# jkflying/opencalibration

Hardware: AMD Instinct MI355X
Metric: images/sec end-to-end (extract+match+relax) on synthetic aerial grid; LM iters/sec (higher is better)
Workload: dtype f32 (extract) + fp4 0/1 bits, f32 accumulate, exact (match) + f64 (RANSAC, relax)

## Files before the change

opencalibration_amd/csrc/match.hip:

```cpp
#include "ctx.hpp"

#include <algorithm>
#include <unordered_map>
#include <vector>

namespace
{

constexpr int BLOCK = 256;
constexpr uint32_t KEY_SHIFT = 20;
constexpr uint32_t KEY_MASK = (1u << KEY_SHIFT) - 1;

__device__ __forceinline__ uint32_t med3_u32(uint32_t a, uint32_t b, uint32_t c)
{
    uint32_t r;
    asm("v_med3_u32 %0, %1, %2, %3" : "=v"(r) : "v"(a), "v"(b), "v"(c));
    return r;
}

__device__ __forceinline__ uint32_t bcnt_acc(uint32_t x, uint32_t acc)
{
    uint32_t r;
    asm("v_bcnt_u32_b32 %0, %1, %2" : "=v"(r) : "v"(x), "v"(acc));
    return r;
}

template <int QPT>
__global__ __launch_bounds__(BLOCK) void hamming_2nn_kernel(const uint32_t *__restrict__ desc,
                                                            const uint64_t *__restrict__ img_off,
                                                            const uint32_t *__restrict__ img_n,
                                                            const ochip_pair *__restrict__ pairs,
                                                            const uint64_t *__restrict__ out_off,
                                                            ochip_match *__restrict__ out, uint32_t chunks_per_pair)
{
    const uint32_t pair = blockIdx.x / chunks_per_pair;
    const uint32_t chunk = blockIdx.x - pair * chunks_per_pair;
    const ochip_pair pr = pairs[pair];
    const uint32_t n1 = img_n[pr.image_1], n2 = img_n[pr.image_2];
    const uint32_t q0 = chunk * (BLOCK * QPT);
    if (q0 >= n1)
        return;
    const uint32_t *__restrict__ Q = desc + img_off[pr.image_1] * 16;
    const uint32_t *__restrict__ R = desc + img_off[pr.image_2] * 16;

    uint32_t q[QPT][16];
    uint32_t best[QPT], second[QPT];
#pragma unroll
    for (int j = 0; j < QPT; j++)
    {
        uint32_t qi = q0 + j * BLOCK + threadIdx.x;
        qi = qi < n1 ? qi : n1 - 1;
        const uint4 *src = reinterpret_cast<const uint4 *>(Q + (size_t)qi * 16);
#pragma unroll
        for (int v = 0; v < 4; v++)
        {
            const uint4 t = src[v];
            q[j][4 * v + 0] = t.x;
            q[j][4 * v + 1] = t.y;
            q[j][4 * v + 2] = t.z;
            q[j][4 * v + 3] = t.w;
        }
        best[j] = 0xFFFFFFFFu;
        second[j] = 0xFFFFFFFFu;
    }

    auto load_row = [&](uint32_t (&rw)[16], uint32_t k) {
        const uint32_t kk = k < n2 ? k : n2 - 1;
        const uint32_t *__restrict__ r = R + (size_t)kk * 16;
#pragma unroll
        for (int w = 0; w < 16; w++)
            rw[w] = r[w];
    };
    auto score_row = [&](const uint32_t (&rw)[16], uint32_t k) {
#pragma unroll
        for (int j = 0; j < QPT; j++)
        {
            uint32_t cnt = 0;
#pragma unroll
            for (int w = 0; w < 16; w++)
                cnt = bcnt_acc(q[j][w] ^ rw[w], cnt);
            const uint32_t key = (cnt << KEY_SHIFT) | k;
            second[j] = med3_u32(best[j], second[j], key);
            best[j] = best[j] < key ? best[j] : key;
        }
    };
    if (n2 > 0)
    {
        uint32_t ra[16], rb[16];
        load_row(ra, 0);
        uint32_t k = 0;
        for (; k + 1 < n2; k += 2)
        {
            load_row(rb, k + 1);
            score_row(ra, k);
            load_row(ra, k + 2);
            score_row(rb, k + 1);
        }
        if (k < n2)
            score_row(ra, k);
    }

    ochip_match *__restrict__ o = out + out_off[pair];
#pragma unroll
    for (int j = 0; j < QPT; j++)
    {
        const uint32_t qi = q0 + j * BLOCK + threadIdx.x;
        if (qi < n1)
        {
            ochip_match m;
            m.best_k = best[j] & KEY_MASK;
            m.best_count = (uint16_t)(best[j] >> KEY_SHIFT);
            m.second_count = second[j] == 0xFFFFFFFFu ? (uint16_t)OCHIP_NO_SECOND : (uint16_t)(second[j] >> KEY_SHIFT);
            o[qi] = m;
        }
    }
}

struct sym_job
{
    uint32_t a, b;
    uint64_t off_ab, off_ba;
    uint64_t part_off;
};

__device__ __forceinline__ void top2_merge(uint32_t &b, uint32_t &s, uint32_t ob, uint32_t os)
{
    const uint32_t lo = b < ob ? b : ob, hi = b < ob ? ob : b, ms = s < os ? s : os;
    b = lo;
    s = hi < ms ? hi : ms;
}

__global__ __launch_bounds__(BLOCK) void hamming_2nn_sym_kernel(const uint32_t *__restrict__ desc, const uint64_t *__restrict__ img_off,
                                                                const uint32_t *__restrict__ img_n, const sym_job *__restrict__ jobs,
                                                                ochip_match *__restrict__ out, uint2 *__restrict__ part,
                                                                uint32_t chunks_per_pair)
{
    __shared__ uint32_t T[4][16 * 65];
    const uint32_t pair = blockIdx.x / chunks_per_pair;
    const uint32_t chunk = blockIdx.x - pair * chunks_per_pair;
    const sym_job jb = jobs[pair];
    const uint32_t nA = img_n[jb.a], nB = img_n[jb.b];
    const uint32_t q0 = chunk * BLOCK;
    if (q0 >= nA)
        return;
    const int lane = threadIdx.x & 63, wv = threadIdx.x >> 6;
    if (q0 + wv * 64 >= nA)
        return;
    const uint32_t *__restrict__ Q = desc + img_off[jb.a] * 16;
    const uint32_t *__restrict__ R = desc + img_off[jb.b] * 16;
    const uint32_t qi = q0 + threadIdx.x;
    const bool q_valid = qi < nA;
    uint32_t q[16];
    {
        const uint4 *src = reinterpret_cast<const uint4 *>(Q + (size_t)(q_valid ? qi : nA - 1) * 16);
#pragma unroll
        for (int v = 0; v < 4; v++)
        {
            const uint4 t = src[v];
            q[4 * v + 0] = t.x;
            q[4 * v + 1] = t.y;
            q[4 * v + 2] = t.z;
            q[4 * v + 3] = t.w;
        }
    }
    uint32_t best = 0xFFFFFFFFu, second = 0xFFFFFFFFu;
    auto load_row = [&](uint32_t (&rw)[16], uint32_t k) {
        const uint32_t kk = k < nB ? k : nB - 1;
        const uint32_t *__restrict__ r = R + (size_t)kk * 16;
#pragma unroll
        for (int w = 0; w < 16; w++)
            rw[w] = r[w];
    };
    auto count_row = [&](const uint32_t (&rw)[16]) {
        uint32_t cnt = 0;
#pragma unroll
        for (int w = 0; w < 16; w++)
            cnt = bcnt_acc(q[w] ^ rw[w], cnt);
        return cnt;
    };
    uint32_t *Tw = T[wv];
    const uint32_t n_tiles = (nB + 31) / 32;
    for (uint32_t jt = 0; jt < n_tiles; jt++)
    {
        const uint32_t k0 = jt * 32;
        uint32_t ra[16], rb[16];
        load_row(ra, k0);
#pragma unroll 4
        for (uint32_t j = 0; j < 32; j += 2)
        {
            load_row(rb, k0 + j + 1);
            const uint32_t c0 = count_row(ra);
            load_row(ra, k0 + j + 2);
            const uint32_t c1 = count_row(rb);
            const uint32_t ka = k0 + j, kb = ka + 1;
            if (ka < nB)
            {
                const uint32_t key = (c0 << KEY_SHIFT) | ka;
                second = med3_u32(best, second, key);
                best = best < key ? best : key;
            }
            if (kb < nB)
            {
                const uint32_t key = (c1 << KEY_SHIFT) | kb;
                second = med3_u32(best, second, key);
                best = best < key ? best : key;
            }
            const uint32_t s0 = (q_valid && ka < nB) ? c0 : 0xFFFFu, s1 = (q_valid && kb < nB) ? c1 : 0xFFFFu;
            Tw[(j >> 1) * 65 + lane] = s0 | (s1 << 16);
        }
        __builtin_amdgcn_fence(__ATOMIC_SEQ_CST, "wavefront");
        __builtin_amdgcn_wave_barrier();
        uint32_t cb = 0xFFFFFFFFu, cs = 0xFFFFFFFFu;
        {
            const uint32_t jj = lane & 31, half = lane >> 5;
            const uint32_t *col = Tw + (jj >> 1) * 65 + half * 32;
            const uint32_t sh = (jj & 1) * 16;
            const uint32_t qbase = q0 + wv * 64 + half * 32;
#pragma unroll 8
            for (uint32_t i = 0; i < 32; i++)
            {
                const uint32_t c = (col[i] >> sh) & 0xFFFFu;
                const uint32_t key = (c << KEY_SHIFT) | (qbase + i);
                cs = med3_u32(cb, cs, key);
                cb = cb < key ? cb : key;
            }
            const uint32_t ob = (uint32_t)__shfl_xor((int)cb, 32), os = (uint32_t)__shfl_xor((int)cs, 32);
            top2_merge(cb, cs, ob, os);
            const uint32_t ref = k0 + jj;
            if (half == 0 && ref < nB)
                part[jb.part_off + (size_t)(chunk * 4 + wv) * nB + ref] = make_uint2(cb, cs);
        }
        __builtin_amdgcn_fence(__ATOMIC_SEQ_CST, "wavefront");
        __builtin_amdgcn_wave_barrier();
    }
    if (q_valid)
    {
        ochip_match m;
        m.best_k = best & KEY_MASK;
        m.best_count = (uint16_t)(best >> KEY_SHIFT);
        m.second_count = second == 0xFFFFFFFFu ? (uint16_t)OCHIP_NO_SECOND : (uint16_t)(second >> KEY_SHIFT);
        out[jb.off_ab + qi] = m;
    }
}

__global__ __launch_bounds__(BLOCK) void sym_merge_kernel(const sym_job *__restrict__ jobs, const uint32_t *__restrict__ img_n,
                                                          const uint2 *__restrict__ part, ochip_match *__restrict__ out)
{
    const sym_job jb = jobs[blockIdx.x];
    const uint32_t nA = img_n[jb.a], nB = img_n[jb.b];
    const uint32_t r = blockIdx.y * BLOCK + threadIdx.x;
    if (r >= nB)
        return;
    uint32_t b = 0xFFFFFFFFu, s = 0xFFFFFFFFu;
    const uint32_t tiles = (nA + 63) / 64;
    for (uint32_t c = 0; c < tiles; c++)
    {
        const uint2 p = part[jb.part_off + (size_t)c * nB + r];
        top2_merge(b, s, p.x, p.y);
    }
    ochip_match m;
    m.best_k = b & KEY_MASK;
    m.best_count = (uint16_t)(b >> KEY_SHIFT);
    m.second_count = (s >> KEY_SHIFT) == 0xFFFu ? (uint16_t)OCHIP_NO_SECOND : (uint16_t)(s >> KEY_SHIFT);
    out[jb.off_ba + r] = m;
}

typedef int v8i __attribute__((ext_vector_type(8)));
typedef float v16f __attribute__((ext_vector_type(16)));
constexpr uint32_t MFMA_MAX_REFS = 8192;
constexpr int MFMA_QT = 2;
constexpr int MFMA_QUERIES = 4 * 32 * MFMA_QT;

__global__ __launch_bounds__(256) void expand_fp4_kernel(const uint32_t *__restrict__ desc, uint64_t first, uint64_t n,
                                                         uint32_t *__restrict__ fp4, float *__restrict__ negpop,
                                                         uint32_t *__restrict__ pop)
{
    const uint64_t f = first + (uint64_t)blockIdx.x * 4 + (threadIdx.x >> 6);
    if (f >= first + n)
        return;
    const int j = threadIdx.x & 63;
    const uint32_t x = (desc[f * 16 + (j >> 2)] >> (8 * (j & 3))) & 0xFFu;
    uint32_t t = (x | (x << 12)) & 0x000F000Fu;
    t = (t | (t << 6)) & 0x03030303u;
    t = (t | (t << 3)) & 0x11111111u;
    fp4[f * 64 + j] = t << 1;
    uint32_t c = (uint32_t)__popc(x);
    for (int off = 32; off >= 1; off >>= 1)
        c += (uint32_t)__shfl_xor((int)c, off);
    if (j == 0)
    {
        pop[f] = c;
        negpop[f] = (float)((512 - (int)c) * 8192);
    }
}

__device__ __forceinline__ float med3_f32(float a, float b, float c)
{
    return __builtin_amdgcn_fmed3f(a, b, c);
}
__device__ __forceinline__ float max_f32(float a, float b)
{
    return __int_as_float(max(__float_as_int(a), __float_as_int(b)));
}

__global__ __launch_bounds__(256) void hamming_2nn_mfma_kernel(const uint4 *__restrict__ fp4, const float *__restrict__ negpop,
                                                               const uint32_t *__restrict__ pop,
                                                               const uint64_t *__restrict__ img_off,
                                                               const uint32_t *__restrict__ img_n,
                                                               const ochip_pair *__restrict__ pairs,
                                                               const uint64_t *__restrict__ out_off,
                                                               ochip_match *__restrict__ out, uint32_t chunks_per_pair)
{
    constexpr int TR = 64;
    __shared__ uint4 tileA[2][TR * 17];
    __shared__ float tileC[2][TR];
    const uint32_t pair = blockIdx.x / chunks_per_pair;
    const uint32_t chunk = blockIdx.x - pair * chunks_per_pair;
    const ochip_pair pr = pairs[pair];
    const uint32_t n1 = img_n[pr.image_1], n2 = img_n[pr.image_2];
    const uint32_t q0 = chunk * MFMA_QUERIES;
    if (q0 >= n1 || n2 == 0)
        return;
    const uint64_t off1 = img_off[pr.image_1], off2 = img_off[pr.image_2];
    const int tid = threadIdx.x, lane = tid & 63, wv = tid >> 6, r = lane & 31, h = lane >> 5;
    constexpr int QT = MFMA_QT;
    v8i Bq[QT][8];
#pragma unroll
    for (int t = 0; t < QT; t++)
    {
        uint32_t qi = q0 + wv * (32 * QT) + t * 32 + r;
        qi = qi < n1 ? qi : n1 - 1;
        const uint4 *src = fp4 + (off1 + qi) * 16;
#pragma unroll
        for (int sidx = 0; sidx < 8; sidx++)
        {
            const uint4 v = src[2 * sidx + h];
            Bq[t][sidx] = v8i{(int)v.x, (int)v.y, (int)v.z, (int)v.w, 0, 0, 0, 0};
        }
    }
    float best[QT], second[QT];
#pragma unroll
    for (int t = 0; t < QT; t++)
        best[t] = second[t] = -1.0f;
    const uint32_t n_tiles = (n2 + TR - 1) / TR;
    const uint4 *gsrc = fp4 + off2 * 16 + tid;
    const float *gneg = negpop + off2 + (tid & 63);
    const int st0 = (tid >> 4) * 17 + (tid & 15);
    auto load_tile = [&](uint32_t jt, uint4 (&p)[4], float &c) {
        if ((jt + 1) * TR <= n2)
        {
#pragma unroll
            for (int i = 0; i < 4; i++)
                p[i] = gsrc[(size_t)jt * (TR * 16) + 256 * i];
            c = gneg[jt * TR] + (float)(8191 - (int)(jt * TR + (uint32_t)(tid & 63)));
        }
        else
        {
#pragma unroll
            for (int i = 0; i < 4; i++)
            {
                const uint32_t k = jt * TR + ((uint32_t)tid >> 4) + 16 * i;
                p[i] = fp4[(off2 + (k < n2 ? k : n2 - 1)) * 16 + (tid & 15)];
            }
            const uint32_t kc = jt * TR + (uint32_t)(tid & 63);
            c = kc < n2 ? negpop[off2 + kc] + (float)(8191 - (int)kc) : -1e9f;
        }
    };
    auto put_tile = [&](int buf, const uint4 (&p)[4], float c) {
#pragma unroll
        for (int i = 0; i < 4; i++)
            tileA[buf][st0 + 16 * 17 * i] = p[i];
        if (tid < TR)
            tileC[buf][tid] = c;
    };
    {
        uint4 p[4];
        float c;
        load_tile(0, p, c);
        put_tile(0, p, c);
    }
    __syncthreads();
    uint4 nx[2][4];
    float nc[2] = {0.0f, 0.0f};
#pragma unroll
    for (int q = 0; q < 2; q++)
#pragma unroll
        for (int i = 0; i < 4; i++)
            nx[q][i] = make_uint4(0, 0, 0, 0);
    if (n_tiles > 1)
        load_tile(1, nx[1], nc[1]);
    auto tile = [&](uint32_t jt, uint4 (&mine)[4], float &mine_c, uint4 (&ahead)[4], float &ahead_c) {
        const int cur = (int)(jt & 1);
        const bool more = jt + 1 < n_tiles;
        if (jt + 2 < n_tiles)
            load_tile(jt + 2, ahead, ahead_c);
        v16f acc[2][QT];
#pragma unroll
        for (int sub = 0; sub < 2; sub++)
        {
#pragma unroll
            for (int gidx = 0; gidx < 4; gidx++)
            {
                const float4 c4 = *reinterpret_cast<const float4 *>(&tileC[cur][32 * sub + 8 * gidx + 4 * h]);
                acc[sub][0][4 * gidx + 0] = c4.x;
                acc[sub][0][4 * gidx + 1] = c4.y;
                acc[sub][0][4 * gidx + 2] = c4.z;
                acc[sub][0][4 * gidx + 3] = c4.w;
            }
#pragma unroll
            for (int t = 1; t < QT; t++)
                acc[sub][t] = acc[sub][0];
        }
        typedef int v4i __attribute__((ext_vector_type(4)));
#pragma unroll
        for (int half = 0; half < 2; half++)
        {
            v4i a[2][4];
#pragma unroll
            for (int sub = 0; sub < 2; sub++)
            {
                const uint4 *arow = &tileA[cur][(32 * sub + r) * 17 + h + 8 * half];
#pragma unroll
                for (int sidx = 0; sidx < 4; sidx++)
                {
                    const uint4 t = arow[2 * sidx];
                    a[sub][sidx] = v4i{(int)t.x, (int)t.y, (int)t.z, (int)t.w};
                }
            }
            asm volatile("" : "+v"(a[0][0]), "+v"(a[0][1]), "+v"(a[0][2]), "+v"(a[0][3]), "+v"(a[1][0]), "+v"(a[1][1]), "+v"(a[1][2]), "+v"(a[1][3]));
#pragma unroll
            for (int sidx = 0; sidx < 4; sidx++)
#pragma unroll
                for (int sub = 0; sub < 2; sub++)
                {
                    const v8i A = v8i{a[sub][sidx].x, a[sub][sidx].y, a[sub][sidx].z, a[sub][sidx].w, 0, 0, 0, 0};
#pragma unroll
                    for (int t = 0; t < QT; t++)
                        acc[sub][t] = __builtin_amdgcn_mfma_scale_f32_32x32x64_f8f6f4(A, Bq[t][4 * half + sidx], acc[sub][t], 4, 4, 0, 141, 0, 127);
                }
        }
#pragma unroll
        for (int sub = 0; sub < 2; sub++)
#pragma unroll
            for (int i = 0; i < 16; i++)
            {
#pragma unroll
                for (int t = 0; t < QT; t++)
                {
                    second[t] = med3_f32(best[t], second[t], acc[sub][t][i]);
                    best[t] = max_f32(best[t], acc[sub][t][i]);
                }
            }
        if (more)
            put_tile(cur ^ 1, mine, mine_c);
        __syncthreads();
    };
    for (uint32_t jt = 0; jt < n_tiles; jt += 2)
    {
        tile(jt, nx[1], nc[1], nx[0], nc[0]);
        if (jt + 1 < n_tiles)
            tile(jt + 1, nx[0], nc[0], nx[1], nc[1]);
    }
    ochip_match *__restrict__ o = out + out_off[pair];
#pragma unroll
    for (int t = 0; t < QT; t++)
    {
        const float ob = __shfl_xor(best[t], 32), os = __shfl_xor(second[t], 32);
        const float hi = fmaxf(best[t], ob), lo = fminf(best[t], ob), ms = fmaxf(second[t], os);
        const float b2 = fmaxf(lo, ms);
        const uint32_t qi = q0 + wv * (32 * QT) + t * 32 + r;
        if (h == 0 && qi < n1)
        {
            const uint32_t pq = pop[off1 + qi];
            const int kb = (int)hi;
            ochip_match m;
            m.best_k = 8191u - ((uint32_t)kb & 8191u);
            m.best_count = (uint16_t)(pq + 512u - ((uint32_t)kb >> 13));
            m.second_count = b2 < 0.0f ? (uint16_t)OCHIP_NO_SECOND : (uint16_t)(pq + 512u - ((uint32_t)(int)b2 >> 13));
            o[qi] = m;
        }
    }
}

}

extern "C"
{

int ochip_match_launch(ochip_ctx *ctx, const ochip_pair *pairs, uint32_t n_pairs, const uint64_t *out_offset,
                       uint64_t out_total)
{
    if (!ctx)
        return OCHIP_EINVAL;
    if (n_pairs && (!pairs || !out_offset))
        return ochip_fail(ctx, OCHIP_EINVAL, "pairs/out_offset is NULL");
    if (!ctx->desc_dev)
        return ochip_fail(ctx, OCHIP_ESTATE, "ochip_descriptors_reserve has not been called");
    OCHIP_HIP(ctx, hipSetDevice(ctx->device));
    ctx->match_out_total = out_total;
    if (n_pairs == 0)
        return OCHIP_OK;

    uint32_t max_n1 = 0;
    for (uint32_t p = 0; p < n_pairs; p++)
    {
        const ochip_pair &pr = pairs[p];
        if (pr.image_1 >= ctx->n_images || pr.image_2 >= ctx->n_images || !ctx->img_set[pr.image_1] ||
            !ctx->img_set[pr.image_2])
            return ochip_fail(ctx, OCHIP_ESTATE, "pair %u references an image that was not uploaded", p);
        if (ctx->img_n[pr.image_2] > KEY_MASK)
            return ochip_fail(ctx, OCHIP_EINVAL, "image %u has %u descriptors; the kernel supports <= %u", pr.image_2,
                              ctx->img_n[pr.image_2], KEY_MASK);
        if (out_offset[p] + ctx->img_n[pr.image_1] > out_total)
            return ochip_fail(ctx, OCHIP_EINVAL, "out_offset[%u] + n1 exceeds out_total", p);
        max_n1 = ctx->img_n[pr.image_1] > max_n1 ? ctx->img_n[pr.image_1] : max_n1;
    }

    static const bool use_mfma = !ochip_test_hook("popcount_match");
    std::vector<ochip_pair> mfma_pairs;
    std::vector<uint64_t> mfma_off;
    uint32_t mfma_max_n1 = 0;
    std::vector<char> claimed(n_pairs, 0);
    if (use_mfma)
        for (uint32_t p = 0; p < n_pairs; p++)
        {
            const uint32_t na = ctx->img_n[pairs[p].image_1], nb = ctx->img_n[pairs[p].image_2];
            if (na == 0 || nb == 0 || nb > MFMA_MAX_REFS)
                continue;
            claimed[p] = 1;
            mfma_pairs.push_back(pairs[p]);
            mfma_off.push_back(out_offset[p]);
            mfma_max_n1 = std::max(mfma_max_n1, na);
            ctx->match_computed += (uint64_t)na * nb;
            ctx->match_delivered += (uint64_t)na * nb;
        }
    const uint32_t n_mfma = (uint32_t)mfma_pairs.size();
    constexpr bool use_sym = true;
    std::vector<sym_job> sym;
    std::vector<ochip_pair> single_pairs;
    std::vector<uint64_t> single_off;
    uint64_t part_total = 0, part_max = 0;
    uint32_t sym_max_na = 0, sym_max_nb = 0;
    std::vector<uint32_t> sym_groups{0};
    {
        std::unordered_map<uint64_t, uint32_t> first;
        if (use_sym)
            for (uint32_t p = 0; p < n_pairs; p++)
                if (!claimed[p])
                    first.emplace(((uint64_t)pairs[p].image_1 << 32) | pairs[p].image_2, p);
        for (uint32_t p = 0; p < n_pairs; p++)
        {
            if (claimed[p])
                continue;
            const uint32_t a = pairs[p].image_1, b = pairs[p].image_2;
            const uint32_t na = ctx->img_n[a], nb = ctx->img_n[b];
            static const uint64_t cap_bytes = getenv("OCHIP_MATCH_SYM_CAP_MB") ? (uint64_t)atoll(getenv("OCHIP_MATCH_SYM_CAP_MB")) << 20 : (8ull << 30);
            const uint64_t need = (uint64_t)((na + 63) / 64) * nb;
            if (use_sym && a != b && na > 0 && nb > 0 && need * sizeof(uint2) <= cap_bytes)
            {
                auto it = first.find(((uint64_t)b << 32) | a);
                if (it != first.end() && it->second != p && !claimed[it->second])
                {
                    claimed[p] = claimed[it->second] = 1;
                    if ((part_total + need) * sizeof(uint2) > cap_bytes)
                    {
                        sym_groups.push_back((uint32_t)sym.size());
                        part_total = 0;
                    }
                    sym.push_back(sym_job{a, b, out_offset[p], out_offset[it->second], part_total});
                    part_total += need;
                    part_max = std::max(part_max, part_total);
                    ctx->match_computed += (uint64_t)na * nb;
                    ctx->match_delivered += 2 * (uint64_t)na * nb;
                    sym_max_na = std::max(sym_max_na, na);
                    sym_max_nb = std::max(sym_max_nb, nb);
                    continue;
                }
            }
            claimed[p] = 1;
            ctx->match_computed += (uint64_t)na * nb;
            ctx->match_delivered += (uint64_t)na * nb;
            single_pairs.push_back(pairs[p]);
            single_off.push_back(out_offset[p]);
        }
    }
    const uint32_t n_single = (uint32_t)single_pairs.size(), n_sym = (uint32_t)sym.size();
    uint32_t max_n1_single = 0;
    for (const ochip_pair &pr : single_pairs)
        max_n1_single = std::max(max_n1_single, ctx->img_n[pr.image_1]);

    OCHIP_TRY(ochip_upload_image_tables(ctx));
    OCHIP_TRY(ctx->pairs_dev.ensure(ctx, n_single + n_mfma));
    OCHIP_TRY(ctx->out_off_dev.ensure(ctx, n_single + n_mfma));
    if (n_mfma)
    {
        OCHIP_TRY(ctx->desc_fp4_dev.ensure(ctx, (size_t)ctx->desc_capacity * 16));
        OCHIP_TRY(ctx->desc_negpop_dev.ensure(ctx, ctx->desc_capacity));
        OCHIP_TRY(ctx->desc_pop_dev.ensure(ctx, ctx->desc_capacity));
        if (ctx->fp4_valid < ctx->desc_used)
        {
            const uint64_t n_new = ctx->desc_used - ctx->fp4_valid;
            hipLaunchKernelGGL(expand_fp4_kernel, dim3((uint32_t)((n_new + 3) / 4)), dim3(256), 0, ctx->stream, ctx->desc_dev,
                               ctx->fp4_valid, n_new, ctx->desc_fp4_dev.as<uint32_t>(), ctx->desc_negpop_dev, ctx->desc_pop_dev);
            ctx->fp4_valid = ctx->desc_used;
        }
        OCHIP_HIP(ctx, hipMemcpyAsync(ctx->pairs_dev + n_single, mfma_pairs.data(), (size_t)n_mfma * sizeof(ochip_pair),
                                      hipMemcpyHostToDevice, ctx->stream));
        OCHIP_HIP(ctx, hipMemcpyAsync(ctx->out_off_dev + n_single, mfma_off.data(), (size_t)n_mfma * 8, hipMemcpyHostToDevice,
                                      ctx->stream));
    }
    OCHIP_TRY(ctx->match_out_dev.ensure(ctx, out_total ? out_total : 1));
    if (n_sym)
    {
        OCHIP_TRY(ctx->sym_jobs_dev.ensure(ctx, (size_t)n_sym * sizeof(sym_job)));
        OCHIP_TRY(ctx->sym_part_dev.ensure(ctx, part_max));
    }
    if (n_single)
    {
        OCHIP_HIP(ctx, hipMemcpyAsync(ctx->pairs_dev, single_pairs.data(), (size_t)n_single * sizeof(ochip_pair), hipMemcpyHostToDevice,
                                      ctx->stream));
        OCHIP_HIP(ctx, hipMemcpyAsync(ctx->out_off_dev, single_off.data(), (size_t)n_single * 8, hipMemcpyHostToDevice, ctx->stream));
    }
    if (n_sym)
        OCHIP_HIP(ctx, hipMemcpyAsync(ctx->sym_jobs_dev, sym.data(), (size_t)n_sym * sizeof(sym_job), hipMemcpyHostToDevice, ctx->stream));
    OCHIP_HIP(ctx, ochip_stream_wait(ctx, ctx->stream));
    if (max_n1 == 0)
        return OCHIP_OK;

    constexpr int qpt = 1;
    const uint32_t chunks = (max_n1_single + BLOCK * qpt - 1) / (BLOCK * qpt);
    const uint64_t blocks = (uint64_t)chunks * n_single;
    const uint32_t sym_chunks = (sym_max_na + BLOCK - 1) / BLOCK;
    const uint64_t sym_blocks = (uint64_t)sym_chunks * n_sym;
    const uint32_t mfma_chunks = (mfma_max_n1 + MFMA_QUERIES - 1) / MFMA_QUERIES;
    const uint64_t mfma_blocks = (uint64_t)mfma_chunks * n_mfma;
    if (blocks > 0x7FFFFFFFull || sym_blocks > 0x7FFFFFFFull || mfma_blocks > 0x7FFFFFFFull)
        return ochip_fail(ctx, OCHIP_EINVAL, "batch too large: %llu workgroups", (unsigned long long)(blocks + sym_blocks + mfma_blocks));
    hipEvent_t e0, e1;
    ochip_prof_begin(ctx, OCHIP_K_MATCH, &e0, &e1);
    if (mfma_blocks)
        hipLaunchKernelGGL(hamming_2nn_mfma_kernel, dim3((uint32_t)mfma_blocks), dim3(256), 0, ctx->stream,
                           ctx->desc_fp4_dev, ctx->desc_negpop_dev, ctx->desc_pop_dev, ctx->img_off_dev, ctx->img_n_dev,
                           ctx->pairs_dev + n_single, ctx->out_off_dev + n_single, ctx->match_out_dev, mfma_chunks);
    auto launch = [&](auto kernel) {
        hipLaunchKernelGGL(kernel, dim3((uint32_t)blocks), dim3(BLOCK), 0, ctx->stream, ctx->desc_dev,
                           ctx->img_off_dev, ctx->img_n_dev, ctx->pairs_dev, ctx->out_off_dev, ctx->match_out_dev,
                           chunks);
    };
    if (blocks)
        launch(hamming_2nn_kernel<1>);
    sym_groups.push_back(n_sym);
    for (size_t gi = 0; gi + 1 < sym_groups.size(); gi++)
    {
        const uint32_t g0 = sym_groups[gi], gn = sym_groups[gi + 1] - g0;
        if (gn == 0)
            continue;
        const sym_job *jobs = ctx->sym_jobs_dev.as<sym_job>() + g0;
        hipLaunchKernelGGL(hamming_2nn_sym_kernel, dim3(sym_chunks * gn), dim3(BLOCK), 0, ctx->stream, ctx->desc_dev, ctx->img_off_dev,
                           ctx->img_n_dev, jobs, ctx->match_out_dev, ctx->sym_part_dev, sym_chunks);
        hipLaunchKernelGGL(sym_merge_kernel, dim3(gn, (sym_max_nb + BLOCK - 1) / BLOCK), dim3(BLOCK), 0, ctx->stream, jobs, ctx->img_n_dev,
                           ctx->sym_part_dev, ctx->match_out_dev);
    }
    ochip_prof_end(ctx, OCHIP_K_MATCH, e0, e1);
    OCHIP_HIP(ctx, hipGetLastError());
    return OCHIP_OK;
}

int ochip_match_fetch(ochip_ctx *ctx, ochip_match *out, uint64_t out_total)
{
    if (!ctx)
        return OCHIP_EINVAL;
    if (out_total != ctx->match_out_total)
        return ochip_fail(ctx, OCHIP_EINVAL, "out_total %llu differs from the launch (%llu)",
                          (unsigned long long)out_total, (unsigned long long)ctx->match_out_total);
    if (out_total == 0)
        return OCHIP_OK;
    if (!out)
        return ochip_fail(ctx, OCHIP_EINVAL, "out is NULL");
    OCHIP_HIP(ctx, hipSetDevice(ctx->device));
    OCHIP_HIP(ctx, hipMemcpyAsync(out, ctx->match_out_dev, (size_t)out_total * sizeof(ochip_match),
                                  hipMemcpyDeviceToHost, ctx->stream));
    OCHIP_HIP(ctx, ochip_stream_wait(ctx, ctx->stream));
    return OCHIP_OK;
}

int ochip_match_batch(ochip_ctx *ctx, const ochip_pair *pairs, uint32_t n_pairs, const uint64_t *out_offset,
                      ochip_match *out)
{
    if (!ctx)
        return OCHIP_EINVAL;
    uint64_t total = 0;
    for (uint32_t p = 0; p < n_pairs; p++)
    {
        if (pairs[p].image_1 >= ctx->n_images)
            return ochip_fail(ctx, OCHIP_EINVAL, "pair %u: image out of range", p);
        const uint64_t end = out_offset[p] + ctx->img_n[pairs[p].image_1];
        total = end > total ? end : total;
    }
    int rc = ochip_match_launch(ctx, pairs, n_pairs, out_offset, total);
    if (rc)
        return rc;
    return ochip_match_fetch(ctx, out, total);
}

}
```

Measured before the change: 4148.

## Compute both match directions in one MFMA pass for symmetric image pairs

Adds a symmetric variant of the MFMA Hamming 2-NN kernel. When both (a,b) and (b,a) are requested, one pass over a×b distances yields the forward best/second and also per-reference top-2 partials. It does this by transposing each wave's accumulator tile through shared memory and merging across waves. A merge kernel then reduces the partials for the reverse direction, removing roughly half the MFMA work for paired requests. In exchange it adds shared-memory traffic, a partial buffer in global memory, an extra merge launch, and a forced two-waves-per-EU occupancy.

Result: faster. 4200 (median of 6 runs) (+1.2%).

```diff
diff --git a/opencalibration_amd/csrc/match.hip b/opencalibration_amd/csrc/match.hip
--- a/opencalibration_amd/csrc/match.hip
+++ b/opencalibration_amd/csrc/match.hip
@@ -244,7 +244,7 @@
 }
 
 __global__ __launch_bounds__(BLOCK) void sym_merge_kernel(const sym_job *__restrict__ jobs, const uint32_t *__restrict__ img_n,
-                                                          const uint2 *__restrict__ part, ochip_match *__restrict__ out)
+                                                          const uint2 *__restrict__ part, ochip_match *__restrict__ out, uint32_t group)
 {
     const sym_job jb = jobs[blockIdx.x];
     const uint32_t nA = img_n[jb.a], nB = img_n[jb.b];
@@ -252,7 +252,7 @@
     if (r >= nB)
         return;
     uint32_t b = 0xFFFFFFFFu, s = 0xFFFFFFFFu;
-    const uint32_t tiles = (nA + 63) / 64;
+    const uint32_t tiles = (nA + group - 1) / group;
     for (uint32_t c = 0; c < tiles; c++)
     {
         const uint2 p = part[jb.part_off + (size_t)c * nB + r];
@@ -270,6 +270,11 @@
 constexpr uint32_t MFMA_MAX_REFS = 8192;
 constexpr int MFMA_QT = 2;
 constexpr int MFMA_QUERIES = 4 * 32 * MFMA_QT;
+
+constexpr int SYM_T_ROWS = 64, SYM_T_STRIDE = 36;
+static_assert(8192 * 1024 + 2 * 8191 < (1 << 24), "the keys of both directions must be exact in fp32");
+static_assert(MFMA_MAX_REFS == 8192, "reference and query index share the key's low 13 bits");
+static_assert(SYM_T_STRIDE % 4 == 0 && (SYM_T_STRIDE / 4) % 2 == 1, "16-byte aligned rows whose starts visit all 16 four-bank slots");
 
 __global__ __launch_bounds__(256) void expand_fp4_kernel(const uint32_t *__restrict__ desc, uint64_t first, uint64_t n,
                                                          uint32_t *__restrict__ fp4, float *__restrict__ negpop,
@@ -303,25 +308,17 @@
     return __int_as_float(max(__float_as_int(a), __float_as_int(b)));
 }
 
-__global__ __launch_bounds__(256) void hamming_2nn_mfma_kernel(const uint4 *__restrict__ fp4, const float *__restrict__ negpop,
-                                                               const uint32_t *__restrict__ pop,
-                                                               const uint64_t *__restrict__ img_off,
-                                                               const uint32_t *__restrict__ img_n,
-                                                               const ochip_pair *__restrict__ pairs,
-                                                               const uint64_t *__restrict__ out_off,
-                                                               ochip_match *__restrict__ out, uint32_t chunks_per_pair)
+template <bool SYM>
+__device__ __forceinline__ void hamming_2nn_mfma_body(const uint4 *__restrict__ fp4, const float *__restrict__ negpop,
+                                                      const uint32_t *__restrict__ pop, const uint64_t off1, const uint64_t off2,
+                                                      const uint32_t n1, const uint32_t n2, const uint32_t q0,
+                                                      ochip_match *__restrict__ o, uint2 *__restrict__ part_row)
 {
     constexpr int TR = 64;
     __shared__ uint4 tileA[2][TR * 17];
     __shared__ float tileC[2][TR];
-    const uint32_t pair = blockIdx.x / chunks_per_pair;
-    const uint32_t chunk = blockIdx.x - pair * chunks_per_pair;
-    const ochip_pair pr = pairs[pair];
-    const uint32_t n1 = img_n[pr.image_1], n2 = img_n[pr.image_2];
-    const uint32_t q0 = chunk * MFMA_QUERIES;
-    if (q0 >= n1 || n2 == 0)
-        return;
-    const uint64_t off1 = img_off[pr.image_1], off2 = img_off[pr.image_2];
+    __shared__ float tileT[SYM ? 4 : 1][SYM ? SYM_T_ROWS * SYM_T_STRIDE : 1];
+    __shared__ uint2 tileP[2][SYM ? 4 : 1][SYM ? TR : 1];
     const int tid = threadIdx.x, lane = tid & 63, wv = tid >> 6, r = lane & 31, h = lane >> 5;
     constexpr int QT = MFMA_QT;
     v8i Bq[QT][8];
@@ -342,7 +339,32 @@
 #pragma unroll
     for (int t = 0; t < QT; t++)
         best[t] = second[t] = -1.0f;
+    float qc[QT];
+    float *const Tw = tileT[SYM ? wv : 0];
+    if constexpr (SYM)
+    {
+#pragma unroll
+        for (int t = 0; t < QT; t++)
+        {
+            const uint32_t qi = q0 + wv * (32 * QT) + t * 32 + r;
+            qc[t] = qi < n1 ? negpop[off1 + qi] + (float)(8191 - (int)qi) : -1e9f;
+        }
+    }
     const uint32_t n_tiles = (n2 + TR - 1) / TR;
+    auto flush = [&](uint32_t j) {
+        if (wv != (int)(j & 3))
+            return;
+        uint2 p = tileP[j & 1][0][lane];
+#pragma unroll
+        for (int w = 1; w < 4; w++)
+        {
+            const uint2 o2 = tileP[j & 1][SYM ? w : 0][lane];
+            top2_merge(p.x, p.y, o2.x, o2.y);
+        }
+        const uint32_t ref = j * TR + (uint32_t)lane;
+        if (ref < n2)
+            part_row[ref] = p;
+    };
     const uint4 *gsrc = fp4 + off2 * 16 + tid;
     const float *gneg = negpop + off2 + (tid & 63);
     const int st0 = (tid >> 4) * 17 + (tid & 15);
@@ -394,6 +416,9 @@
         const bool more = jt + 1 < n_tiles;
         if (jt + 2 < n_tiles)
             load_tile(jt + 2, ahead, ahead_c);
+        if constexpr (SYM)
+            if (jt > 0)
+                flush(jt - 1);
         v16f acc[2][QT];
 #pragma unroll
         for (int sub = 0; sub < 2; sub++)
@@ -451,6 +476,51 @@
                     best[t] = max_f32(best[t], acc[sub][t][i]);
                 }
             }
+        if constexpr (SYM)
+        {
+            float cb = -1.0f, cs = -1.0f;
+#pragma unroll
+            for (int t = 0; t < QT; t++)
+            {
+#pragma unroll
+                for (int sub = 0; sub < 2; sub++)
+#pragma unroll
+                    for (int i = 0; i < 16; i++)
+                        Tw[(32 * sub + (i & 3) + 8 * (i >> 2) + 4 * h) * SYM_T_STRIDE + r] = acc[sub][t][i] + qc[t];
+                __builtin_amdgcn_fence(__ATOMIC_SEQ_CST, "wavefront");
+                __builtin_amdgcn_wave_barrier();
+                const float4 *row = reinterpret_cast<const float4 *>(Tw + lane * SYM_T_STRIDE);
+#pragma unroll
+                for (int jb = 0; jb < 8; jb += 4)
+                {
+                    float4 v[4];
+#pragma unroll
+                    for (int j = 0; j < 4; j++)
+                        v[j] = row[jb + j];
+#pragma unroll
+                    for (int j = 0; j < 4; j++)
+                    {
+                        cs = med3_f32(cb, cs, v[j].x);
+                        cb = max_f32(cb, v[j].x);
+                        cs = med3_f32(cb, cs, v[j].y);
+                        cb = max_f32(cb, v[j].y);
+                        cs = med3_f32(cb, cs, v[j].z);
+                        cb = max_f32(cb, v[j].z);
+                        cs = med3_f32(cb, cs, v[j].w);
+                        cb = max_f32(cb, v[j].w);
+                    }
+                    asm volatile("" : "+v"(cb), "+v"(cs));
+                }
+                __builtin_amdgcn_fence(__ATOMIC_SEQ_CST, "wavefront");
+                __builtin_amdgcn_wave_barrier();
+            }
+            const float kc = (float)(8191 - (int)(jt * TR + (uint32_t)lane));
+            const uint32_t vb = (uint32_t)(int)(cb - kc), vs = (uint32_t)(int)(cs - kc);
+            uint2 p;
+            p.x = cb < 0.0f ? 0xFFFFFFFFu : ((1024u - (vb >> 13)) << KEY_SHIFT) | (8191u - (vb & 8191u));
+            p.y = cs < 0.0f ? 0xFFFFFFFFu : ((1024u - (vs >> 13)) << KEY_SHIFT) | (8191u - (vs & 8191u));
+            tileP[cur][wv][lane] = p;
+        }
         if (more)
             put_tile(cur ^ 1, mine, mine_c);
         __syncthreads();
@@ -461,7 +531,8 @@
         if (jt + 1 < n_tiles)
             tile(jt + 1, nx[0], nc[0], nx[1], nc[1]);
     }
-    ochip_match *__restrict__ o = out + out_off[pair];
+    if constexpr (SYM)
+        flush(n_tiles - 1);
 #pragma unroll
     for (int t = 0; t < QT; t++)
     {
@@ -480,6 +551,42 @@
             o[qi] = m;
         }
     }
+}
+
+__global__ __launch_bounds__(256) void hamming_2nn_mfma_kernel(const uint4 *__restrict__ fp4, const float *__restrict__ negpop,
+                                                               const uint32_t *__restrict__ pop,
+                                                               const uint64_t *__restrict__ img_off,
+                                                               const uint32_t *__restrict__ img_n,
+                                                               const ochip_pair *__restrict__ pairs,
+                                                               const uint64_t *__restrict__ out_off,
+                                                               ochip_match *__restrict__ out, uint32_t chunks_per_pair)
+{
+    const uint32_t pair = blockIdx.x / chunks_per_pair;
+    const uint32_t chunk = blockIdx.x - pair * chunks_per_pair;
+    const ochip_pair pr = pairs[pair];
+    const uint32_t n1 = img_n[pr.image_1], n2 = img_n[pr.image_2];
+    const uint32_t q0 = chunk * MFMA_QUERIES;
+    if (q0 >= n1 || n2 == 0)
+        return;
+    hamming_2nn_mfma_body<false>(fp4, negpop, pop, img_off[pr.image_1], img_off[pr.image_2], n1, n2, q0, out + out_off[pair], nullptr);
+}
+
+__global__ __launch_bounds__(256) __attribute__((amdgpu_waves_per_eu(2, 2))) void hamming_2nn_sym_mfma_kernel(const uint4 *__restrict__ fp4, const float *__restrict__ negpop,
+                                                                   const uint32_t *__restrict__ pop,
+                                                                   const uint64_t *__restrict__ img_off,
+                                                                   const uint32_t *__restrict__ img_n,
+                                                                   const sym_job *__restrict__ jobs, ochip_match *__restrict__ out,
+                                                                   uint2 *__restrict__ part, uint32_t chunks_per_pair)
+{
+    const uint32_t pair = blockIdx.x / chunks_per_pair;
+    const uint32_t chunk = blockIdx.x - pair * chunks_per_pair;
+    const sym_job jb = jobs[pair];
+    const uint32_t n1 = img_n[jb.a], n2 = img_n[jb.b];
+    const uint32_t q0 = chunk * MFMA_QUERIES;
+    if (q0 >= n1 || n2 == 0)
+        return;
+    hamming_2nn_mfma_body<true>(fp4, negpop, pop, img_off[jb.a], img_off[jb.b], n1, n2, q0, out + jb.off_ab,
+                                part + jb.part_off + (size_t)chunk * n2);
 }
 
 }
@@ -516,30 +623,70 @@
         max_n1 = ctx->img_n[pr.image_1] > max_n1 ? ctx->img_n[pr.image_1] : max_n1;
     }
 
+    static const uint64_t cap_bytes = getenv("OCHIP_MATCH_SYM_CAP_MB") ? (uint64_t)atoll(getenv("OCHIP_MATCH_SYM_CAP_MB")) << 20 : (8ull << 30);
+    uint64_t part_max = 0;
+
     static const bool use_mfma = !ochip_test_hook("popcount_match");
+    static const bool mfma_sym = !ochip_test_hook("mfma_one_direction");
     std::vector<ochip_pair> mfma_pairs;
     std::vector<uint64_t> mfma_off;
-    uint32_t mfma_max_n1 = 0;
+    std::vector<sym_job> msym;
+    std::vector<uint32_t> msym_groups{0};
+    uint32_t mfma_max_n1 = 0, msym_max_na = 0, msym_max_nb = 0;
     std::vector<char> claimed(n_pairs, 0);
     if (use_mfma)
+    {
+        auto fits = [&](uint32_t p) {
+            const uint32_t na = ctx->img_n[pairs[p].image_1], nb = ctx->img_n[pairs[p].image_2];
+            return na != 0 && nb != 0 && nb <= MFMA_MAX_REFS;
+        };
+        std::unordered_map<uint64_t, uint32_t> first;
+        if (mfma_sym)
+            for (uint32_t p = 0; p < n_pairs; p++)
+                if (fits(p))
+                    first.emplace(((uint64_t)pairs[p].image_1 << 32) | pairs[p].image_2, p);
+        uint64_t part_total = 0;
         for (uint32_t p = 0; p < n_pairs; p++)
         {
-            const uint32_t na = ctx->img_n[pairs[p].image_1], nb = ctx->img_n[pairs[p].image_2];
-            if (na == 0 || nb == 0 || nb > MFMA_MAX_REFS)
+            if (claimed[p] || !fits(p))
                 continue;
+            const uint32_t a = pairs[p].image_1, b = pairs[p].image_2;
+            const uint32_t na = ctx->img_n[a], nb = ctx->img_n[b];
             claimed[p] = 1;
+            ctx->match_computed += (uint64_t)na * nb;
+            const uint64_t need = (uint64_t)((na + MFMA_QUERIES - 1) / MFMA_QUERIES) * nb;
+            if (mfma_sym && a != b && na <= MFMA_MAX_REFS && need * sizeof(uint2) <= cap_bytes)
+            {
+                auto it = first.find(((uint64_t)b << 32) | a);
+                if (it != first.end() && !claimed[it->second])
+                {
+                    claimed[it->second] = 1;
+                    if ((part_total + need) * sizeof(uint2) > cap_bytes)
+                    {
+                        msym_groups.push_back((uint32_t)msym.size());
+                        part_total = 0;
+                    }
+                    msym.push_back(sym_job{a, b, out_offset[p], out_offset[it->second], part_total});
+                    part_total += need;
+                    part_max = std::max(part_max, part_total);
+                    ctx->match_delivered += 2 * (uint64_t)na * nb;
+                    msym_max_na = std::max(msym_max_na, na);
+                    msym_max_nb = std::max(msym_max_nb, nb);
+                    continue;
+                }
+            }
             mfma_pairs.push_back(pairs[p]);
             mfma_off.push_back(out_offset[p]);
             mfma_max_n1 = std::max(mfma_max_n1, na);
-            ctx->match_computed += (uint64_t)na * nb;
             ctx->match_delivered += (uint64_t)na * nb;
         }
-    const uint32_t n_mfma = (uint32_t)mfma_pairs.size();
+    }
+    const uint32_t n_mfma = (uint32_t)mfma_pairs.size(), n_msym = (uint32_t)msym.size();
     constexpr bool use_sym = true;
     std::vector<sym_job> sym;
     std::vector<ochip_pair> single_pairs;
     std::vector<uint64_t> single_off;
-    uint64_t part_total = 0, part_max = 0;
+    uint64_t part_total = 0;
     uint32_t sym_max_na = 0, sym_max_nb = 0;
     std::vector<uint32_t> sym_groups{0};
     {
@@ -554,7 +701,6 @@
                 continue;
             const uint32_t a = pairs[p].image_1, b = pairs[p].image_2;
             const uint32_t na = ctx->img_n[a], nb = ctx->img_n[b];
-            static const uint64_t cap_bytes = getenv("OCHIP_MATCH_SYM_CAP_MB") ? (uint64_t)atoll(getenv("OCHIP_MATCH_SYM_CAP_MB")) << 20 : (8ull << 30);
             const uint64_t need = (uint64_t)((na + 63) / 64) * nb;
             if (use_sym && a != b && na > 0 && nb > 0 && need * sizeof(uint2) <= cap_bytes)
             {
@@ -592,7 +738,7 @@
     OCHIP_TRY(ochip_upload_image_tables(ctx));
     OCHIP_TRY(ctx->pairs_dev.ensure(ctx, n_single + n_mfma));
     OCHIP_TRY(ctx->out_off_dev.ensure(ctx, n_single + n_mfma));
-    if (n_mfma)
+    if (n_mfma + n_msym)
     {
         OCHIP_TRY(ctx->desc_fp4_dev.ensure(ctx, (size_t)ctx->desc_capacity * 16));
         OCHIP_TRY(ctx->desc_negpop_dev.ensure(ctx, ctx->desc_capacity));
@@ -604,15 +750,18 @@
                                ctx->fp4_valid, n_new, ctx->desc_fp4_dev.as<uint32_t>(), ctx->desc_negpop_dev, ctx->desc_pop_dev);
             ctx->fp4_valid = ctx->desc_used;
         }
+    }
+    if (n_mfma)
+    {
         OCHIP_HIP(ctx, hipMemcpyAsync(ctx->pairs_dev + n_single, mfma_pairs.data(), (size_t)n_mfma * sizeof(ochip_pair),
                                       hipMemcpyHostToDevice, ctx->stream));
         OCHIP_HIP(ctx, hipMemcpyAsync(ctx->out_off_dev + n_single, mfma_off.data(), (size_t)n_mfma * 8, hipMemcpyHostToDevice,
                                       ctx->stream));
     }
     OCHIP_TRY(ctx->match_out_dev.ensure(ctx, out_total ? out_total : 1));
-    if (n_sym)
-    {
-        OCHIP_TRY(ctx->sym_jobs_dev.ensure(ctx, (size_t)n_sym * sizeof(sym_job)));
+    if (n_sym + n_msym)
+    {
+        OCHIP_TRY(ctx->sym_jobs_dev.ensure(ctx, (size_t)(n_sym + n_msym) * sizeof(sym_job)));
         OCHIP_TRY(ctx->sym_part_dev.ensure(ctx, part_max));
     }
     if (n_single)
@@ -623,6 +772,9 @@
     }
     if (n_sym)
         OCHIP_HIP(ctx, hipMemcpyAsync(ctx->sym_jobs_dev, sym.data(), (size_t)n_sym * sizeof(sym_job), hipMemcpyHostToDevice, ctx->stream));
+    if (n_msym)
+        OCHIP_HIP(ctx, hipMemcpyAsync(ctx->sym_jobs_dev.as<sym_job>() + n_sym, msym.data(), (size_t)n_msym * sizeof(sym_job),
+                                      hipMemcpyHostToDevice, ctx->stream));
     OCHIP_HIP(ctx, ochip_stream_wait(ctx, ctx->stream));
     if (max_n1 == 0)
         return OCHIP_OK;
@@ -634,14 +786,30 @@
     const uint64_t sym_blocks = (uint64_t)sym_chunks * n_sym;
     const uint32_t mfma_chunks = (mfma_max_n1 + MFMA_QUERIES - 1) / MFMA_QUERIES;
     const uint64_t mfma_blocks = (uint64_t)mfma_chunks * n_mfma;
-    if (blocks > 0x7FFFFFFFull || sym_blocks > 0x7FFFFFFFull || mfma_blocks > 0x7FFFFFFFull)
-        return ochip_fail(ctx, OCHIP_EINVAL, "batch too large: %llu workgroups", (unsigned long long)(blocks + sym_blocks + mfma_blocks));
+    const uint32_t msym_chunks = (msym_max_na + MFMA_QUERIES - 1) / MFMA_QUERIES;
+    const uint64_t msym_blocks = (uint64_t)msym_chunks * n_msym;
+    if (blocks > 0x7FFFFFFFull || sym_blocks > 0x7FFFFFFFull || mfma_blocks > 0x7FFFFFFFull || msym_blocks > 0x7FFFFFFFull)
+        return ochip_fail(ctx, OCHIP_EINVAL, "batch too large: %llu workgroups",
+                          (unsigned long long)(blocks + sym_blocks + mfma_blocks + msym_blocks));
     hipEvent_t e0, e1;
     ochip_prof_begin(ctx, OCHIP_K_MATCH, &e0, &e1);
     if (mfma_blocks)
         hipLaunchKernelGGL(hamming_2nn_mfma_kernel, dim3((uint32_t)mfma_blocks), dim3(256), 0, ctx->stream,
                            ctx->desc_fp4_dev, ctx->desc_negpop_dev, ctx->desc_pop_dev, ctx->img_off_dev, ctx->img_n_dev,
                            ctx->pairs_dev + n_single, ctx->out_off_dev + n_single, ctx->match_out_dev, mfma_chunks);
+    msym_groups.push_back(n_msym);
+    for (size_t gi = 0; gi + 1 < msym_groups.size(); gi++)
+    {
+        const uint32_t g0 = msym_groups[gi], gn = msym_groups[gi + 1] - g0;
+        if (gn == 0)
+            continue;
+        const sym_job *jobs = ctx->sym_jobs_dev.as<sym_job>() + n_sym + g0;
+        hipLaunchKernelGGL(hamming_2nn_sym_mfma_kernel, dim3(msym_chunks * gn), dim3(256), 0, ctx->stream, ctx->desc_fp4_dev,
+                           ctx->desc_negpop_dev, ctx->desc_pop_dev, ctx->img_off_dev, ctx->img_n_dev, jobs, ctx->match_out_dev,
+                           ctx->sym_part_dev, msym_chunks);
+        hipLaunchKernelGGL(sym_merge_kernel, dim3(gn, (msym_max_nb + BLOCK - 1) / BLOCK), dim3(BLOCK), 0, ctx->stream, jobs, ctx->img_n_dev,
+                           ctx->sym_part_dev, ctx->match_out_dev, (uint32_t)MFMA_QUERIES);
+    }
     auto launch = [&](auto kernel) {
         hipLaunchKernelGGL(kernel, dim3((uint32_t)blocks), dim3(BLOCK), 0, ctx->stream, ctx->desc_dev,
                            ctx->img_off_dev, ctx->img_n_dev, ctx->pairs_dev, ctx->out_off_dev, ctx->match_out_dev,
@@ -659,7 +827,7 @@
         hipLaunchKernelGGL(hamming_2nn_sym_kernel, dim3(sym_chunks * gn), dim3(BLOCK), 0, ctx->stream, ctx->desc_dev, ctx->img_off_dev,
                            ctx->img_n_dev, jobs, ctx->match_out_dev, ctx->sym_part_dev, sym_chunks);
         hipLaunchKernelGGL(sym_merge_kernel, dim3(gn, (sym_max_nb + BLOCK - 1) / BLOCK), dim3(BLOCK), 0, ctx->stream, jobs, ctx->img_n_dev,
-                           ctx->sym_part_dev, ctx->match_out_dev);
+                           ctx->sym_part_dev, ctx->match_out_dev, 64u);
     }
     ochip_prof_end(ctx, OCHIP_K_MATCH, e0, e1);
     OCHIP_HIP(ctx, hipGetLastError());
```
